# andewx/dieselfluid

Hardware: AMD Instinct MI355X
Metric: M particle-steps/sec, 16M-particle WCSPH dam-break; % HBM roofline (higher is better)
Workload: dtype f32; 1 GPU; WCSPH dam-break, 16003008 particles (n3=252), h=2dx, uniform-grid neighbours, density + pressure/viscosity force + integrate + walls, math=fast; particles=16003008, parallelism=single GPU

## Files before the change

### dieselfluid_amd/csrc/kernels_skin.hpp

```cpp
#pragma once

#include "kernels_tiled.hpp"

namespace dsl {

constexpr int kLEntries = 8;
constexpr int kLMaxChunks = 12;
constexpr int kLMaxEntries = kLMaxChunks * kLEntries - 1;
constexpr int kLBlock = 512;
constexpr unsigned int kLGlobal = 0xffffu;
constexpr float kSkinTauSteps = 16.0f;
constexpr int kLQuads = 14;
static_assert(kTRows * kLQuads <= kLBlock, "one quad per lane");

__global__ void k_skin_decide(SkinState* st) {
  const float d = __builtin_sqrtf(__uint_as_float(st->disp2_bits)) * (1.0f + 1.0e-6f);
  const bool rb = st->force != 0 || !(d <= st->budget);
  st->rebuild = rb ? 1 : 0;
  if (st->unlisted * 64 > st->n_live) st->give_up = 1;
  if (rb) {
    st->ids_sel ^= 1;
    st->n_rebuilds += 1;
    st->unlisted = 0;
    st->fields_own = st->fields_padded = 0u;
    const float vmax = __builtin_sqrtf(__uint_as_float(st->vmax2_bits)) * (1.0f + 1.0e-6f);
    float tau = 0.0f;
    if (st->predict > 0.0f && vmax > 0.0f && vmax < 3.0e38f) tau = fminf(st->predict * st->budget / vmax, kSkinTauSteps * st->dt);
    st->tau = tau;
  }
  st->disp = d;
  st->force = 0;
  st->disp2_bits = 0u;
  st->vmax2_bits = 0u;
  st->n_steps += 1;
  st->history = (st->history << 1) | (rb ? 1u : 0u);
  if (st->n_steps >= 16 && __builtin_popcount(st->history & 0xffffu) >= 5) st->give_up = 1;
}

__device__ __forceinline__ unsigned int pad_entry(const TileMeta& m) { return (unsigned int)(m.row_lds[1] - kTPad) << 4; }

__global__ __launch_bounds__(kLBlock) void k_list_build_v1(DevConsts c, TileGrid tg, const int* __restrict__ desc_of,
                                                        const int* __restrict__ n_tiles, const int* __restrict__ desc,
                                                        const unsigned int* __restrict__ nmask, int mstride,
                                                        uint4* __restrict__ lists, int lstride, SkinState* st,
                                                        SkinGate gate, CSoa3 p, float wide_thr) {
  if (gate.closed()) return;
  __shared__ TileMeta metas[2];
  constexpr int kLStaged = 8;
  __shared__ uint4 held[kLStaged][kLBlock];
  __shared__ unsigned int tile_fields[2];
  const int tid = threadIdx.x;
  if (tid < 2) tile_fields[tid] = 0u;
  TileFeed feed(desc_of, *n_tiles);
  int di = 0;
  bool have = feed.pop(di);
  if (have) tile_meta_store(metas[0], tile_meta_request(desc, di));
  for (int cur = 0; have; cur ^= 1) {
    const TileMeta& m = metas[cur];
    sync_lds();
    have = feed.pop(di);
    int table_word = 0;
    if (have) table_word = tile_meta_request(desc, di);
    const int ntarg = m.tprefix[kTB * kTB];
    const unsigned int pad = pad_entry(m);
    if (m.overflow != 0 && tid == 0) atomicAdd(&st->unlisted, ntarg);
    for_each_target<true, kLBlock>(ntarg, tid, tid, [&](auto shared_c, int t, int sub, int k) {
      constexpr bool SHARED = decltype(shared_c)::value;
      if (SHARED && sub != 0) return;
      const TileTarget tt = tile_target(m, t);
      const int g = tt.g;
      unsigned int b0 = 0u, b1 = 0u, b2 = 0u, b3 = 0u;
      int n = 0;
      auto push = [&](unsigned int entry) {
        b0 = __builtin_amdgcn_alignbit(b1, b0, 16);
        b1 = __builtin_amdgcn_alignbit(b2, b1, 16);
        b2 = __builtin_amdgcn_alignbit(b3, b2, 16);
        b3 = (b3 >> 16) | (entry << 16);
        n += 1;
        if ((n & (kLEntries - 1)) == 0) {
          const int ch = (n >> 3) - 1;
          if (ch < kLStaged) held[ch][tid] = make_uint4(b0, b1, b2, b3);
          else if (ch < kLMaxChunks) lists[(size_t)ch * lstride + g] = make_uint4(b0, b1, b2, b3);
        }
      };
      auto emit = [&](int rec) {
        if (rec != tt.own) push((unsigned int)rec << 4);
      };
      const bool masks = m.overflow == 0;
      if (masks) {
        int rj[9], rje[9];
        unsigned int w1[9], w2[9];
#pragma unroll
        for (int ri = 0; ri < 9; ++ri) {
          tile_run(m, tt.srow + (ri / 3 - 1) * kTH + (ri % 3 - 1), tt.lx, rj[ri], rje[ri]);
          const int len = rje[ri] - rj[ri];
          w1[ri] = (len > 0 && len <= 64) ? nmask[(size_t)ri * mstride + g] : 0u;
          w2[ri] = (len > 32 && len <= 64) ? nmask[(size_t)(kMaskHigh + ri) * mstride + g] : 0u;
        }
        push(0u);
#pragma unroll
        for (int ri = 0; ri < 9; ++ri) {
          const int j = rj[ri], je = rje[ri], len = je - j;
          if (len > 64) {
            const int rr = tt.srow + (ri / 3 - 1) * kTH + (ri % 3 - 1);
            const int g0 = m.row_gs[rr] - m.row_lds[rr];
            const float xi = p.x[g], yi = p.y[g], zi = p.z[g];
            for (int r = j; r < je; ++r) {
              const float dx = xi - p.x[g0 + r], dy = yi - p.y[g0 + r], dz = zi - p.z[g0 + r];
              const float tq = __builtin_fmaf(-dist2<true>(dx, dy, dz), c.inv_hh, 1.0f);
              if (tq > wide_thr) emit(r);
            }
            continue;
          }
          unsigned int w = w1[ri];
          int top = j + ((min(len, 32) + 3) & ~3) - 1;
          while (w != 0u) {
            const int b = __builtin_ctz(w);
            w &= w - 1u;
            emit(top - b);
          }
          w = w2[ri];
          top = j + 32 + ((len - 32 + 3) & ~3) - 1;
          while (w != 0u) {
            const int b = __builtin_ctz(w);
            w &= w - 1u;
            emit(top - b);
          }
        }
      }
      const bool fits = masks && n <= kLMaxChunks * kLEntries;
      if (masks && !fits) st->list_overflow = 1;
      int fields = fits ? n : 0;
      const int own_fields = fields;
      if constexpr (!SHARED) {
        int wmax = 0;
#pragma unroll
        for (int bit = 6; bit >= 0; --bit) {
          const int cand = wmax | (1 << bit);
          if (__builtin_amdgcn_ballot_w64(fields >= cand) != 0ull) wmax = cand;
        }
        fields = wmax;
      }
      atomicAdd(&tile_fields[0], (unsigned int)own_fields);
      atomicAdd(&tile_fields[1], (unsigned int)(fits ? fields : 0));
      const int nch = (fields + kLEntries - 1) / kLEntries;
      if (fits)
        while (n < nch * kLEntries) push(pad);
      for (int ch = 0; ch < min(nch, kLStaged); ++ch) {
        uint4 v = held[ch][tid];
        if (ch == 0) v.x = (v.x & 0xffff0000u) | (unsigned int)fields;
        if (fits) lists[(size_t)ch * lstride + g] = v;
      }
      if (!fits) lists[g] = make_uint4(kLGlobal, 0u, 0u, 0u);
    });
    if (have) tile_meta_store(metas[cur ^ 1], table_word);
    sync_lds();
    if (tid == 0) {
      atomicAdd(&st->fields_own, tile_fields[0]);
      atomicAdd(&st->fields_padded, tile_fields[1]);
      tile_fields[0] = tile_fields[1] = 0u;
    }
  }
}

constexpr int kLQueue = 24;
__global__ __launch_bounds__(kLBlock, 4) void k_list_build(DevConsts c, TileGrid tg, const int* __restrict__ desc_of,
                                                        const int* __restrict__ n_tiles, const int* __restrict__ desc,
                                                        const unsigned int* __restrict__ nmask, int mstride,
                                                        uint4* __restrict__ lists, int lstride, SkinState* st,
                                                        SkinGate gate, CSoa3 p, float wide_thr) {
  if (gate.closed()) return;
  __shared__ TileMeta metas[2];
  __shared__ unsigned int qword[kLQueue][kLBlock];
  __shared__ unsigned short qtop[kLQueue][kLBlock];
  __shared__ unsigned int tile_fields[2];
  const int tid = threadIdx.x;
  if (tid < 2) tile_fields[tid] = 0u;
  TileFeed feed(desc_of, *n_tiles);
  int di = 0;
  bool have = feed.pop(di);
  if (have) tile_meta_store(metas[0], tile_meta_request(desc, di));
  for (int cur = 0; have; cur ^= 1) {
    const TileMeta& m = metas[cur];
    sync_lds();
    have = feed.pop(di);
    int table_word = 0;
    if (have) table_word = tile_meta_request(desc, di);
    const int ntarg = m.tprefix[kTB * kTB];
    const unsigned int pad = pad_entry(m);
    if (m.overflow != 0 && tid == 0) atomicAdd(&st->unlisted, ntarg);
    for_each_target<true, kLBlock>(ntarg, tid, tid, [&](auto shared_c, int t, int sub, int k) {
      constexpr bool SHARED = decltype(shared_c)::value;
      if (SHARED && sub != 0) return;
      const TileTarget tt = tile_target(m, t);
      const int g = tt.g;
      const bool masks = m.overflow == 0;
      int nq = 0, total = 0;
      bool too_many = false;
      auto enqueue = [&](unsigned int w, int top) {
        if (w != 0u) {
          if (nq < kLQueue) {
            qword[nq][tid] = w;
            qtop[nq][tid] = (unsigned short)top;
          } else {
            too_many = true;
          }
          nq += 1;
          total += __builtin_popcount(w);
        }
      };
      if (masks) {
        unsigned int run[9], w1[9], w2[9];
        unsigned int unmasked = 0u;
#pragma unroll
        for (int ri = 0; ri < 9; ++ri) {
          run[ri] = (unsigned int)m.run[(tt.srow + (ri / 3 - 1) * kTH + (ri % 3 - 1)) * kTB + tt.lx - 1];
          const int len = (int)(run[ri] >> 16) - (int)(run[ri] & 0xffffu);
          w1[ri] = (len > 0 && len <= 64) ? nmask[(size_t)ri * mstride + g] : 0u;
          w2[ri] = (len > 32 && len <= 64) ? nmask[(size_t)(kMaskHigh + ri) * mstride + g] : 0u;
          if (len > 64) unmasked |= 1u << ri;
        }
#pragma unroll
        for (int ri = 0; ri < 9; ++ri) {
          const int j = (int)(run[ri] & 0xffffu), len = (int)(run[ri] >> 16) - j;
          unsigned int a = w1[ri], b = w2[ri];
          const int top1 = j + ((min(len, 32) + 3) & ~3) - 1;
          const int top2 = j + 32 + ((len - 32 + 3) & ~3) - 1;
          if (ri == 4) {
            const int b1 = top1 - tt.own, b2 = top2 - tt.own;
            if (b1 >= 0 && b1 < 32) a &= ~(1u << b1);
            if (b2 >= 0 && b2 < 32) b &= ~(1u << b2);
          }
          enqueue(a, top1);
          enqueue(b, top2);
        }
        while (unmasked != 0u) {
          const int ri = __builtin_ctz(unmasked);
          unmasked &= unmasked - 1u;
          const int rr = tt.srow + (ri / 3 - 1) * kTH + (ri % 3 - 1);
          int j, je;
          tile_run(m, rr, tt.lx, j, je);
          const int g0 = m.row_gs[rr] - m.row_lds[rr];
          const float xi = p.x[g], yi = p.y[g], zi = p.z[g];
          for (int r0 = j; r0 < je; r0 += 32) {
            unsigned int w = 0u;
            const int top = r0 + 31;
            for (int r = r0; r < min(r0 + 32, je); ++r) {
              const float dx = xi - p.x[g0 + r], dy = yi - p.y[g0 + r], dz = zi - p.z[g0 + r];
              const float tq = __builtin_fmaf(-dist2<true>(dx, dy, dz), c.inv_hh, 1.0f);
              if (tq > wide_thr && r != tt.own) w |= 1u << (top - r);
            }
            enqueue(w, top);
          }
        }
      }
      const int n_own = 1 + total;
      const bool fits = masks && !too_many && n_own <= kLMaxChunks * kLEntries;
      if (masks && !fits) st->list_overflow = 1;
      int fields = fits ? n_own : 0;
      const int own_fields = fields;
      int wmax = 0;
#pragma unroll
      for (int bit = 6; bit >= 0; --bit) {
        const int cand = wmax | (1 << bit);
        if (__builtin_amdgcn_ballot_w64(fields >= cand) != 0ull) wmax = cand;
      }
      if constexpr (!SHARED) fields = fits ? wmax : 0;
      atomicAdd(&tile_fields[0], (unsigned int)own_fields);
      atomicAdd(&tile_fields[1], (unsigned int)fields);
      const int nch = (fields + kLEntries - 1) / kLEntries;
      const int nch_wave = (wmax + kLEntries - 1) / kLEntries;
      unsigned int b0 = 0u, b1 = 0u, b2 = 0u, b3 = 0u;
      unsigned int k0 = 0u, k1 = 0u, k2 = 0u, k3 = 0u;
      int qi = 0;
      unsigned int w = 0u, top = 0u;
      unsigned int wn = (fits && nq > 0) ? qword[0][tid] : 0u, tn = (fits && nq > 0) ? qtop[0][tid] : 0u;
      const int nq_live = fits ? nq : 0;
      for (int it = 0; it < nch_wave * kLEntries; ++it) {
        unsigned int entry = pad;
        if (it == 0) {
          entry = 0u;
        } else {
          if (w == 0u && qi < nq_live) {
            w = wn;
            top = tn;
            qi += 1;
            if (qi < nq_live) {
              wn = qword[qi][tid];
              tn = qtop[qi][tid];
            }
          }
          if (w != 0u) {
            const int b = __builtin_ctz(w);
            w &= w - 1u;
            entry = (top - (unsigned int)b) << 4;
          }
        }
        b0 = __builtin_amdgcn_alignbit(b1, b0, 16);
        b1 = __builtin_amdgcn_alignbit(b2, b1, 16);
        b2 = __builtin_amdgcn_alignbit(b3, b2, 16);
        b3 = (b3 >> 16) | (entry << 16);
        if ((it & (kLEntries - 1)) == kLEntries - 1) {
          const int ch = it >> 3;
          if (ch == 0) {
            k0 = b0, k1 = b1, k2 = b2, k3 = b3;
          } else if (ch < nch) {
            lists[(size_t)ch * lstride + g] = make_uint4(b0, b1, b2, b3);
          }
        }
      }
      if (fits) lists[g] = make_uint4((k0 & 0xffff0000u) | (unsigned int)fields, k1, k2, k3);
      else lists[g] = make_uint4(kLGlobal, 0u, 0u, 0u);
    });
    if (have) tile_meta_store(metas[cur ^ 1], table_word);
    sync_lds();
    if (tid == 0) {
      atomicAdd(&st->fields_own, tile_fields[0]);
      atomicAdd(&st->fields_padded, tile_fields[1]);
      tile_fields[0] = tile_fields[1] = 0u;
    }
  }
}

template <int NF, bool DEALT, class Load4, class Store>
__device__ __forceinline__ void stage_tile(const TileMeta& m, Load4&& load4, Store&& store) {
  if constexpr (DEALT) {
    const int nq = __builtin_amdgcn_readfirstlane((int)m.qprefix[kTRows]);
    auto pass = [&](int base) {
      StageRegs<NF> sr;
      const StageWhere w = stage_issue_dealt<NF>(m, load4, sr, base + (int)threadIdx.x, nq);
      stage_commit_dealt<NF>(sr, w, store);
    };
    pass(0);
    for (int base = kLBlock; base < nq; base += kLBlock) pass(base);
    stage_pads<NF>(m, store, threadIdx.x);
    return;
  }
  const int t = threadIdx.x, r = t / kLQuads, k = t - r * kLQuads;
  if (r >= kTRows) return;
  const int len = m.row_len[r], gs = m.row_gs[r], ls = m.row_lds[r];
  for (int q = k; 4 * q < len; q += kLQuads) {
    float4 v[NF];
    load4(gs + 4 * q, v);
#pragma unroll
    for (int i = 0; i < 4; ++i) {
      if (4 * q + i < len) {
        float rec[NF];
#pragma unroll
        for (int a = 0; a < NF; ++a) rec[a] = f4_at(v[a], i);
        store(ls + 4 * q + i, rec, true);
      }
    }
  }
  const int npad = m.row_lds[r + 1] - ls - len;
  if (k < npad) {
    float rec[NF];
#pragma unroll
    for (int a = 0; a < NF; ++a) rec[a] = 0.0f;
    store(ls + len + k, rec, false);
  }
}

__device__ __forceinline__ const float4& lds_at(const float4* base, unsigned int byte_offset) {
  return *reinterpret_cast<const float4*>(reinterpret_cast<const char*>(base) + byte_offset);
}

struct Chunk {
  unsigned int x, y, z, w;
};
__device__ __forceinline__ Chunk load_chunk(const uint4* __restrict__ lists, size_t index) {
  const uint4 v = lists[index];
  return Chunk{v.x, v.y, v.z, v.w};
}
__device__ __forceinline__ Chunk pad_chunk(unsigned int pad) {
  const unsigned int w = pad | (pad << 16);
  return Chunk{w, w, w, w};
}
__device__ __forceinline__ unsigned int take_count(Chunk& e, unsigned int pad) {
  const unsigned int cnt = e.x & 0xffffu;
  e.x = (e.x & 0xffff0000u) | pad;
  return cnt;
}
__device__ __forceinline__ int chunks_of(unsigned int cnt) { return cnt == kLGlobal ? 0 : (int)((cnt + kLEntries) >> 3); }

template <class Body>
__device__ __forceinline__ void walk_shared(const uint4* __restrict__ lists, int lstride, int g, unsigned int pad, int sub,
                                            int k, unsigned int fields, Body&& body) {
  const int nch = fields == kLGlobal ? 0 : (int)((fields + kLEntries - 1) >> 3);
  for (int ch = sub; __builtin_amdgcn_ballot_w64(ch < nch) != 0ull; ch += k) {
    Chunk e = pad_chunk(pad);
    if (ch < nch) e = load_chunk(lists, (size_t)ch * lstride + g);
    if (ch == 0) e.x = (e.x & 0xffff0000u) | pad;
    body(e);
  }
}
__device__ __forceinline__ unsigned int shared_fields(const uint4* __restrict__ lists, int g, int sub) {
  unsigned int f = 0u;
  if (sub == 0) f = lists[g].x & 0xffffu;
  return (unsigned int)__shfl((int)f, (int)((threadIdx.x & (kWave - 1)) - sub), kWave);
}

__global__ __launch_bounds__(kLBlock, 4) void k_density_list(DevConsts c, TileGrid tg, const int* __restrict__ desc_of,
                                                             const int* __restrict__ n_tiles, const int* __restrict__ desc,
                                                             const int* __restrict__ cell_start, const SkinState* st,
                                                             CSoa3 pX, CSoa3 pZ, const uint4* __restrict__ lists,
                                                             int lstride, float* __restrict__ rho,
                                                             float* __restrict__ pterm) {
  __shared__ TileMeta metas[2];
  __shared__ float4 A[kTCap];
  const int tid = threadIdx.x;
  const CSoa3 p = st->rebuild ? pZ : pX;
  TileFeed feed(desc_of, *n_tiles);
  int di = 0;
  bool have = feed.pop(di);
  if (have) tile_meta_store(metas[0], tile_meta_request(desc, di));
  for (int cur = 0; have; cur ^= 1) {
    const TileMeta& m = metas[cur];
    sync_lds();
    have = feed.pop(di);
    int table_word = 0;
    if (have) table_word = tile_meta_request(desc, di);
    const int ntarg = m.tprefix[kTB * kTB];
    const bool staged = m.overflow == 0;
    const unsigned int pad = pad_entry(m);
    Chunk q0 = pad_chunk(pad), q1 = q0;
    const bool first_full = ntarg > kLBlock / 2;
    TileTarget tt0{0, 0, 0, 0};
    const int tperm = (tid & ~(kWave - 1)) + b128_group_slot(tid & (kWave - 1));
    if (first_full && tperm < ntarg) {
      tt0 = tile_target(m, tperm);
      q0 = load_chunk(lists, tt0.g);
      q1 = load_chunk(lists, (size_t)lstride + tt0.g);
    }
    if (staged) stage_tile<3, (kStageDealt & 1) != 0>(m, LoadPos4{p}, StoreTileRecord(A, m, c.inv_hh));
    if (have) tile_meta_store(metas[cur ^ 1], table_word);
    sync_lds();
    for_each_target<true, kLBlock>(ntarg, tid, tperm, [&](auto shared_c, int t, int sub, int k) {
      constexpr bool SHARED = decltype(shared_c)::value;
      TileTarget tt;
      unsigned int fields;
      if constexpr (SHARED) {
        tt = tile_target(m, t);
        fields = shared_fields(lists, tt.g, sub);
      } else {
        if (t == tperm) tt = tt0;
        else {
          tt = tile_target(m, t);
          q0 = load_chunk(lists, tt.g);
          q1 = load_chunk(lists, (size_t)lstride + tt.g);
        }
        fields = take_count(q0, pad);
      }
      const int g = tt.g;
      float acc = 0.0f;
      if (staged && fields != kLGlobal) {
        const float4 me = A[tt.own];
        const float two_hh = 2.0f * c.inv_hh;
        const float sx = two_hh * me.x, sy = two_hh * me.y, sz = two_hh * me.z, a0 = 1.0f + me.w;
        float acc0 = 0.0f, acc1 = 0.0f;
        float4 cq[4];
        auto fetch4 = [&](unsigned int w0, unsigned int w1) {
          cq[0] = lds_at(A, w0 & 0xffffu);
          cq[1] = lds_at(A, w0 >> 16);
          cq[2] = lds_at(A, w1 & 0xffffu);
          cq[3] = lds_at(A, w1 >> 16);
        };
        auto sum4 = [&](const float4 (&r)[4]) {
#pragma unroll
          for (int u = 0; u < 4; ++u) {
            const float q = fma_clamp01(r[u].z, sz, __builtin_fmaf(r[u].y, sy, __builtin_fmaf(r[u].x, sx, r[u].w + a0)));
            if (u & 1) acc1 = __builtin_fmaf(q, q, acc1);
            else acc0 = __builtin_fmaf(q, q, acc0);
          }
        };
        if constexpr (SHARED) {
          walk_shared(lists, lstride, g, pad, sub, k, fields, [&](const Chunk& e) {
            fetch4(e.x, e.y);
            float4 c1[4] = {cq[0], cq[1], cq[2], cq[3]};
            fetch4(e.z, e.w);
            sum4(c1);
            sum4(cq);
          });
        } else {
          const int nf = __builtin_amdgcn_readfirstlane((int)fields), nch = (nf + kLEntries - 1) >> 3;
          const uint4* lp = lists + (size_t)2 * lstride + g;
          Chunk e = q0, e1 = q1;
          fetch4(e.x, e.y);
          for (int ch = 0;;) {
            float4 c1[4] = {cq[0], cq[1], cq[2], cq[3]};
            fetch4(e.z, e.w);
            sum4(c1);
            if (8 * ch + 4 >= nf) break;
            const Chunk en = e1;
            if (ch + 2 < nch) e1 = load_chunk(lp, 0);
            lp += lstride;
            float4 c2[4] = {cq[0], cq[1], cq[2], cq[3]};
            fetch4(en.x, en.y);
            sum4(c2);
            e = en;
            ch += 1;
            if (8 * ch >= nf) break;
          }
        }
        acc = acc0 + acc1;
      } else if (sub == 0) {
        const float xi = p.x[g], yi = p.y[g], zi = p.z[g];
        float a = 0.0f;
        for_each_grid_candidate(c, cell_start, xi, yi, zi, [&](int j) {
          if (j == g) return;
          const float dx = xi - p.x[j], dy = yi - p.y[j], dz = zi - p.z[j];
          const float r2 = dist2<true>(dx, dy, dz);
          if (r2 < c.hh) {
            const float q = __builtin_fmaf(-r2, c.inv_hh, 1.0f);
            a = __builtin_fmaf(q, q, a);
          }
        });
        acc = a;
      }
      if constexpr (SHARED) {
        for (int o = 1; o < k; o <<= 1) acc += __shfl_xor(acc, o, kWave);
        if (sub != 0) return;
      }
      acc *= c.mass * c.A;
      rho[g] = acc;
      const float pr = tait_eos<true>(c, acc, c.eos_d0_grad);
      pterm[g] = acc > 0.0f ? dsl_div<true>(pr, acc * acc) : 0.0f;
    });
  }
}

template <bool WANT_G, bool WANT_V, bool QUEUE>
__global__ __launch_bounds__(kLBlock, 4) void k_force_list(DevConsts c, TileGrid tg, const int* __restrict__ desc_of,
                                                           const int* __restrict__ n_tiles, const int* __restrict__ desc,
                                                           const int* __restrict__ cell_start, SkinState* st, CSoa3 pX,
                                                           CSoa3 vX, CSoa3 pZ, CSoa3 vZ, CSoa3 pR, const float* __restrict__ rho,
                                                           const float* __restrict__ pterm,
                                                           const uint4* __restrict__ lists, int lstride, Soa3 pout,
                                                           Soa3 vout, DevStats* stats, int* __restrict__ walk_ctr) {
  __shared__ TileMeta metas[2];
  __shared__ float4 A[kTCap];
  __shared__ float4 B[kTCap];
  __shared__ int feed_slot[2];
  const int tid = threadIdx.x;
  const bool rb = st->rebuild != 0;
  const CSoa3 pin = rb ? pZ : pX, vin = rb ? vZ : vX;
  unsigned int vbits = 0u, fbits = 0u, dbits = 0u;
  typename TileSource<QUEUE>::type feed = TileSource<QUEUE>::make(desc_of, *n_tiles, walk_ctr, feed_slot);
  int di = 0;
  bool have = feed.pop(di);
  if (have) tile_meta_store(metas[0], tile_meta_request(desc, di));
  for (int cur = 0; have; cur ^= 1) {
    const TileMeta& m = metas[cur];
    sync_lds();
    have = feed.pop(di);
    int table_word = 0;
    if (have) table_word = tile_meta_request(desc, di);
    const int ntarg = m.tprefix[kTB * kTB];
    const bool staged = m.overflow == 0;
    const unsigned int pad = pad_entry(m);
    Chunk q0 = pad_chunk(pad), q1 = q0;
    const bool first_full = ntarg > kLBlock / 2;
    TileTarget tt0{0, 0, 0, 0};
    const int tperm = (tid & ~(kWave - 1)) + b128_group_slot(tid & (kWave - 1));
    if (first_full && tperm < ntarg) {
      tt0 = tile_target(m, tperm);
      q0 = load_chunk(lists, tt0.g);
      q1 = load_chunk(lists, (size_t)lstride + tt0.g);
    }
    if (staged)
      stage_tile<8, (kStageDealt & 2) != 0>(
          m,
          [&](int gg, float4* o) {
            o[0] = load4u(pin.x + gg);
            o[1] = load4u(pin.y + gg);
            o[2] = load4u(pin.z + gg);
            o[3] = WANT_G ? load4u(pterm + gg) : make_float4(0.f, 0.f, 0.f, 0.f);
            if constexpr (WANT_V) {
              o[4] = load4u(vin.x + gg);
              o[5] = load4u(vin.y + gg);
              o[6] = load4u(vin.z + gg);
              o[7] = load4u(rho + gg);
            } else {
              o[4] = o[5] = o[6] = o[7] = make_float4(0.f, 0.f, 0.f, 0.f);
            }
          },
          [&](int slot, const float* o, bool real) {
            float4 a = make_float4(kFar, kFar, kFar, 0.f), b = make_float4(0.f, 0.f, 0.f, 0.f);
            if (real && o[0] == o[0] && o[1] == o[1] && o[2] == o[2]) {
              a = make_float4(o[0], o[1], o[2], o[3]);
              if constexpr (WANT_V) b = make_float4(o[4], o[5], o[6], o[7] > 0.0f ? __builtin_amdgcn_rcpf(o[7]) : 0.0f);
            }
            A[slot] = a;
            if constexpr (WANT_V) B[slot] = b;
          });
    if (have) tile_meta_store(metas[cur ^ 1], table_word);
    sync_lds();
    for_each_target<true, kLBlock>(ntarg, tid, tperm, [&](auto shared_c, int t, int sub, int k) {
      constexpr bool SHARED = decltype(shared_c)::value;
      TileTarget tt;
      unsigned int fields;
      if constexpr (SHARED) {
        tt = tile_target(m, t);
        fields = shared_fields(lists, tt.g, sub);
      } else {
        if (t == tperm) tt = tt0;
        else {
          tt = tile_target(m, t);
          q0 = load_chunk(lists, tt.g);
          q1 = load_chunk(lists, (size_t)lstride + tt.g);
        }
        fields = take_count(q0, pad);
      }
      const int g = tt.g;
      float px, py, pz, vx, vy, vz;
      float gx = 0.f, gy = 0.f, gz = 0.f, lx_ = 0.f, ly_ = 0.f, lz_ = 0.f, lw_ = 0.f;
      const bool listed = staged && fields != kLGlobal;
      if (listed) {
        const float4 a = A[tt.own];
        px = a.x, py = a.y, pz = a.z;
        const float pti = WANT_G ? a.w : 0.f;
        if (px == kFar) px = py = pz = __uint_as_float(0x7fc00000u);
        if constexpr (WANT_V) {
          const float4 b = B[tt.own];
          vx = b.x, vy = b.y, vz = b.z;
        } else {
          vx = vin.x[g], vy = vin.y[g], vz = vin.z[g];
        }
        if constexpr (WANT_G || WANT_V) {
          const float ninvh = -c.inv_h;
          auto accum = [&](const float4& ra, const float4& rb2) {
            const float dx = ra.x - px, dyy = ra.y - py, dzz = ra.z - pz;
            float r2 = __builtin_fmaf(dzz, dzz, __builtin_fmaf(dyy, dyy, dx * dx));
            r2 = fmaxf(r2, 1.0e-30f);
            const float rinv = __builtin_amdgcn_rsqf(r2);
            const float dist = r2 * rinv;
            const float q = fma1_clamp01_uniform(dist, ninvh);
            if constexpr (WANT_G) {
              const float kk = (q * q) * (pti + ra.w) * rinv;
              gx = __builtin_fmaf(dx, kk, gx);
              gy = __builtin_fmaf(dyy, kk, gy);
              gz = __builtin_fmaf(dzz, kk, gz);
            }
            if constexpr (WANT_V) {
              const float w = q * rb2.w;
              lx_ = __builtin_fmaf(rb2.x, w, lx_);
              ly_ = __builtin_fmaf(rb2.y, w, ly_);
              lz_ = __builtin_fmaf(rb2.z, w, lz_);
              lw_ += w;
            }
          };
          struct Pair1 {
            float4 a, b;
          };
          auto fetch1 = [&](unsigned int off) {
            Pair1 r;
            r.a = lds_at(A, off);
            r.b = r.a;
            if constexpr (WANT_V) r.b = lds_at(B, off);
            return r;
          };
          if constexpr (SHARED) {
            walk_shared(lists, lstride, g, pad, sub, k, fields, [&](const Chunk& e) {
              const unsigned int w[4] = {e.x, e.y, e.z, e.w};
#pragma unroll
              for (int u = 0; u < 4; ++u) {
                const Pair1 r0 = fetch1(w[u] & 0xffffu), r1 = fetch1(w[u] >> 16);
                accum(r0.a, r0.b);
                accum(r1.a, r1.b);
              }
            });
          } else {
            const int nf = __builtin_amdgcn_readfirstlane((int)fields), nch = (nf + kLEntries - 1) >> 3;
            const uint4* lp = lists + (size_t)2 * lstride + g;
            Chunk e = q0, e1 = q1;
            Pair1 p0 = fetch1(e.x & 0xffffu), p1 = fetch1(e.x >> 16);
            auto word = [&](unsigned int next_word) {
              Pair1 cu = p0;
              p0 = fetch1(next_word & 0xffffu);
              accum(cu.a, cu.b);
              cu = p1;
              p1 = fetch1(next_word >> 16);
              accum(cu.a, cu.b);
            };
            for (int ch = 0;;) {
              word(e.y);
              if (8 * ch + 2 >= nf) break;
              word(e.z);
              if (8 * ch + 4 >= nf) break;
              word(e.w);
              if (8 * ch + 6 >= nf) break;
              const Chunk en = e1;
              if (ch + 2 < nch) e1 = load_chunk(lp, 0);
              lp += lstride;
              word(en.x);
              e = en;
              ch += 1;
              if (8 * ch >= nf) break;
            }
          }
        }
      } else {
        px = pin.x[g], py = pin.y[g], pz = pin.z[g];
        vx = vin.x[g], vy = vin.y[g], vz = vin.z[g];
        if (sub == 0) {
          float accG[3] = {0.f, 0.f, 0.f}, accV[3] = {0.f, 0.f, 0.f};
          if constexpr (WANT_G || WANT_V)
            force_sweep<true, WANT_G, WANT_V>(c, grid_neigh(cell_start), g, pin, vin, rho, pterm, accG, accV, nullptr, nullptr);
          gx = accG[0], gy = accG[1], gz = accG[2];
          lx_ = accV[0], ly_ = accV[1], lz_ = accV[2];
        }
      }
      if constexpr (SHARED) {
        for (int o = 1; o < k; o <<= 1) {
          gx += __shfl_xor(gx, o, kWave);
          gy += __shfl_xor(gy, o, kWave);
          gz += __shfl_xor(gz, o, kWave);
          lx_ += __shfl_xor(lx_, o, kWave);
          ly_ += __shfl_xor(ly_, o, kWave);
          lz_ += __shfl_xor(lz_, o, kWave);
          lw_ += __shfl_xor(lw_, o, kWave);
        }
        if (sub != 0) return;
      }
      if (listed) {
        if constexpr (WANT_V) {
          lx_ = __builtin_fmaf(-vx, lw_, lx_);
          ly_ = __builtin_fmaf(-vy, lw_, ly_);
          lz_ = __builtin_fmaf(-vz, lw_, lz_);
        }
        const float sg = -c.B;
        gx *= sg;
        gy *= sg;
        gz *= sg;
        const float sv = c.C * c.mass;
        lx_ *= sv;
        ly_ *= sv;
        lz_ *= sv;
      }
      float fx = c.reset[0], fy = c.reset[1], fz = c.reset[2];
      if constexpr (WANT_G) {
        const float dm = rho[g] * c.mass * c.pressure_sign;
        fx = __builtin_fmaf(gx, dm, fx);
        fy = __builtin_fmaf(gy, dm, fy);
        fz = __builtin_fmaf(gz, dm, fz);
      }
      if constexpr (WANT_V) {
        fx = __builtin_fmaf(lx_, c.mu, fx);
        fy = __builtin_fmaf(ly_, c.mu, fy);
        fz = __builtin_fmaf(lz_, c.mu, fz);
      }
      fx += c.ext[0];
      fy += c.ext[1];
      fz += c.ext[2];
      integrate_core(c, fx, fy, fz, px, py, pz, vx, vy, vz, vbits, fbits);
      {
        const float ex = px - pR.x[g], ey = py - pR.y[g], ez = pz - pR.z[g];
        const unsigned int db = nonneg_bits(__builtin_fmaf(ez, ez, __builtin_fmaf(ey, ey, ex * ex)));
        dbits = db > dbits ? db : dbits;
      }
      pout.x[g] = px;
      pout.y[g] = py;
      pout.z[g] = pz;
      vout.x[g] = vx;
      vout.y[g] = vy;
      vout.z[g] = vz;
    });
  }
  feed.finish();
  wave_atomic_max(&stats->max_vel_bits, vbits);
  wave_atomic_max(&stats->max_f_bits, fbits);
  wave_atomic_max(&st->disp2_bits, dbits);
  wave_atomic_max(&st->vmax2_bits, vbits);
}

}
```

Before: 8324 M particle-steps/s.

## Fully unroll force list walk with 3-slot chunk ring and raise occupancy

Replaces the rolled neighbour-list loop in the unshared force path with a fully unrolled loop over the maximum chunk count. A three-entry register ring issues chunk loads two ahead, and sched barriers stop the compiler from reordering the LDS fetches behind the accumulation. For the pressure-only variant it also raises the launch-bounds waves-per-EU hint from 4 to 6. The aim is to hide global and LDS latency and improve occupancy, at the cost of more code size, tighter register limits that may cause spills, and the opaque-pointer asm tricks.

```diff
diff --git a/dieselfluid_amd/csrc/kernels_skin.hpp b/dieselfluid_amd/csrc/kernels_skin.hpp
--- a/dieselfluid_amd/csrc/kernels_skin.hpp
+++ b/dieselfluid_amd/csrc/kernels_skin.hpp
@@ -12,6 +12,11 @@
 constexpr float kSkinTauSteps = 16.0f;
 constexpr int kLQuads = 14;
 static_assert(kTRows * kLQuads <= kLBlock, "one quad per lane");
+#ifndef DSL_LIST_WALK
+#define DSL_LIST_WALK 2
+#endif
+constexpr int kListWalk = DSL_LIST_WALK;
+constexpr int force_list_waves(bool want_v) { return (kListWalk & 2) != 0 && !want_v ? 6 : 4; }
 
 __global__ void k_skin_decide(SkinState* st) {
   const float d = __builtin_sqrtf(__uint_as_float(st->disp2_bits)) * (1.0f + 1.0e-6f);
@@ -381,6 +386,43 @@
   e.x = (e.x & 0xffff0000u) | pad;
   return cnt;
 }
+__device__ __forceinline__ void loads_issued() {
+  asm volatile("" ::: "memory");
+  __builtin_amdgcn_sched_barrier(0);
+}
+typedef unsigned int ListWords __attribute__((ext_vector_type(4)));
+typedef const __attribute__((address_space(1))) ListWords* ListPtr;
+__device__ __forceinline__ unsigned long long unknown_pointer(const uint4* p) {
+  unsigned long long a = reinterpret_cast<unsigned long long>(p);
+  asm volatile("" : "+v"(a));
+  return a;
+}
+__device__ __forceinline__ unsigned long long unknown_pointer_uniform(const uint4* p) {
+  unsigned long long a = reinterpret_cast<unsigned long long>(p);
+  asm volatile("" : "+s"(a));
+  return a;
+}
+struct ChunkRing {
+  Chunk c[3];
+  unsigned long long next;
+  unsigned long long last;
+  int lstride, nch;
+  __device__ __forceinline__ ChunkRing(const uint4* __restrict__ lists, int lstride_, int g, int nch_, const Chunk& q0,
+                                       const Chunk& q1)
+      : next(unknown_pointer(lists + (size_t)2 * lstride_ + g)),
+        last(unknown_pointer_uniform(lists + (size_t)max(nch_ - 1, 0) * lstride_ + __builtin_amdgcn_readfirstlane(g))),
+        lstride(lstride_), nch(nch_) {
+    c[0] = q0;
+    c[1] = q1;
+  }
+  __device__ __forceinline__ void request(int ch) {
+    if (ch + 2 >= kLMaxChunks) return;
+    const ListWords v = *(ListPtr)(ch + 2 < nch ? next : last);
+    c[(ch + 2) % 3] = Chunk{v.x, v.y, v.z, v.w};
+    next += (unsigned long long)lstride * sizeof(uint4);
+  }
+  __device__ __forceinline__ const Chunk& at(int ch) const { return c[ch % 3]; }
+};
 __device__ __forceinline__ int chunks_of(unsigned int cnt) { return cnt == kLGlobal ? 0 : (int)((cnt + kLEntries) >> 3); }
 
 template <class Body>
@@ -530,7 +572,7 @@
 }
 
 template <bool WANT_G, bool WANT_V, bool QUEUE>
-__global__ __launch_bounds__(kLBlock, 4) void k_force_list(DevConsts c, TileGrid tg, const int* __restrict__ desc_of,
+__global__ __launch_bounds__(kLBlock, force_list_waves(WANT_V)) void k_force_list(DevConsts c, TileGrid tg, const int* __restrict__ desc_of,
                                                            const int* __restrict__ n_tiles, const int* __restrict__ desc,
                                                            const int* __restrict__ cell_start, SkinState* st, CSoa3 pX,
                                                            CSoa3 vX, CSoa3 pZ, CSoa3 vZ, CSoa3 pR, const float* __restrict__ rho,
@@ -670,32 +712,57 @@
               }
             });
           } else {
+            constexpr bool kStraight = (kListWalk & 2) != 0;
             const int nf = __builtin_amdgcn_readfirstlane((int)fields), nch = (nf + kLEntries - 1) >> 3;
-            const uint4* lp = lists + (size_t)2 * lstride + g;
-            Chunk e = q0, e1 = q1;
-            Pair1 p0 = fetch1(e.x & 0xffffu), p1 = fetch1(e.x >> 16);
+            Pair1 p0 = fetch1(q0.x & 0xffffu), p1 = fetch1(q0.x >> 16);
             auto word = [&](unsigned int next_word) {
               Pair1 cu = p0;
               p0 = fetch1(next_word & 0xffffu);
+              if constexpr (kStraight) loads_issued();
               accum(cu.a, cu.b);
               cu = p1;
               p1 = fetch1(next_word >> 16);
+              if constexpr (kStraight) loads_issued();
               accum(cu.a, cu.b);
             };
-            for (int ch = 0;;) {
-              word(e.y);
-              if (8 * ch + 2 >= nf) break;
-              word(e.z);
-              if (8 * ch + 4 >= nf) break;
-              word(e.w);
-              if (8 * ch + 6 >= nf) break;
-              const Chunk en = e1;
-              if (ch + 2 < nch) e1 = load_chunk(lp, 0);
-              lp += lstride;
-              word(en.x);
-              e = en;
-              ch += 1;
-              if (8 * ch >= nf) break;
+            if constexpr (kStraight) {
+              ChunkRing ring(lists, lstride, g, nch, q0, q1);
+#pragma unroll
+              for (int ch = 0; ch < kLMaxChunks; ++ch) {
+                ring.request(ch);
+                const Chunk& e = ring.at(ch);
+                word(e.y);
+                if (8 * ch + 2 >= nf) break;
+                word(e.z);
+                if (8 * ch + 4 >= nf) break;
+                word(e.w);
+                if (8 * ch + 6 >= nf) break;
+                if (ch + 1 == kLMaxChunks) {
+                  accum(p0.a, p0.b);
+                  accum(p1.a, p1.b);
+                  break;
+                }
+                word(ring.at(ch + 1).x);
+                if (8 * ch + 8 >= nf) break;
+              }
+            } else {
+              const uint4* lp = lists + (size_t)2 * lstride + g;
+              Chunk e = q0, e1 = q1;
+              for (int ch = 0;;) {
+                word(e.y);
+                if (8 * ch + 2 >= nf) break;
+                word(e.z);
+                if (8 * ch + 4 >= nf) break;
+                word(e.w);
+                if (8 * ch + 6 >= nf) break;
+                const Chunk en = e1;
+                if (ch + 2 < nch) e1 = load_chunk(lp, 0);
+                lp += lstride;
+                word(en.x);
+                e = en;
+                ch += 1;
+                if (8 * ch >= nf) break;
+              }
             }
           }
         }
```

Result: faster. 8440 M particle-steps/s (median of 6 runs) (+1.4%).
